# Lymphatus/caesium-clt

Measured on AMD Instinct MI355X. Metric: megapixels/sec JPEG q=80 1920x1080 batch, higher is better.
Workload: dtype int32

## Files before the change

### caesium-clt_amd/csrc/k_aclist.hip

```cpp
#include "kernels.h"
#include "wave.h"
#include "tok_bits.h"

namespace csh {

#define CSH_LP_WORDS 1024

__device__ __forceinline__ static uint32_t lbitlen(uint32_t v) { return 32u - uint32_t(__clz(v)); }
__device__ __forceinline__ static int lwave() { return int(threadIdx.x) / CSP_WAVE_THREADS; }

#define CSH_NZ_HALF 16
__device__ __forceinline__ static uint4 nz_load(const EncCtx &c, const NzSet &S, uint32_t u, int bx, int by, uint32_t oct) {
    uint4 q; q.x = q.y = q.z = q.w = 0u;
    if (u < S.nunits) {
        const int b = by * S.bw + bx;
        q = *reinterpret_cast<const uint4 *>(c.coef + (size_t(S.tile_base) + size_t(b >> 6)) * CSH_TILE_I16 + size_t((b & 63) * CSH_BLK_STRIDE) + size_t(oct) * CSH_OCT_STRIDE);
    }
    return q;
}
__device__ __forceinline__ static uint32_t nz_mask8(const uint4 &q, uint32_t oct) {
    uint32_t m = 0;
    m |= (q.x & 0xFFFFu) ? 1u : 0u;   m |= (q.x >> 16) ? 2u : 0u;
    m |= (q.y & 0xFFFFu) ? 4u : 0u;   m |= (q.y >> 16) ? 8u : 0u;
    m |= (q.z & 0xFFFFu) ? 16u : 0u;  m |= (q.z >> 16) ? 32u : 0u;
// ... 279 lines not shown
    const uint32_t idx = blockIdx.x * 4u + uint32_t(wv);
    if (idx >= c.nlist_runs) return;
    const uint32_t cs0 = c.list_runs[idx];
    const SlotRec r = c.slots[cs0];
    if (c.work_active && !c.work_active[r.work]) return;
    const uint32_t nrun = run_chunks(c, r);
    const uint64_t lbase = c.nzlists[r.nzlist].base;
    ListSlot nx = list_chunk(c, lbase, r.nzrec);
    uint32_t *hist = &s_hist[wv][0][0], *flag = s_flag[wv];
    LFOR(l) {
        uint4 zero; zero.x = zero.y = zero.z = zero.w = 0u;
        for (int i = 4 * l; i < 1024; i += 256) *reinterpret_cast<uint4 *>(hist + i) = zero;
        if (l < 16) flag[l] = 0u;
    }
    CSP_WAVE_SYNC();
    const uint32_t Ss = r.Ss, Se = r.Se;
    LV<uint32_t> freq[4];
    LFOR(l) { freq[0][l] = 0u; freq[1][l] = 0u; freq[2][l] = 0u; freq[3][l] = 0u; }
    LV<uint32_t> x0, x1, x2, x3;
    bool ahead = false;
    for (uint32_t ci = 0; ci < nrun; ci++) {
        const ListSlot ls = nx;
        const bool more = ci + 1u < nrun;
        if (more) nx = list_chunk(c, lbase, r.nzrec + ci + 1u);
        if (!ahead) LFOR(l) list_load4(ls, 4u * uint32_t(l), x0[l], x1[l], x2[l], x3[l]);
        ahead = false;
        uint32_t carry = CSH_NZ_END;
        LV<uint32_t> raw;
        LFOR(l) raw[l] = 0u;
        for (uint32_t g0 = 0; g0 < ls.n; g0 += 256) {
            const LV<uint32_t> e0 = x0, e1 = x1, e2 = x2, e3 = x3;
            if (g0 + 256u < ls.n) LFOR(l) list_load4(ls, g0 + 256u + 4u * uint32_t(l), x0[l], x1[l], x2[l], x3[l]);
            else if (more) { LFOR(l) list_load4(nx, 4u * uint32_t(l), x0[l], x1[l], x2[l], x3[l]); ahead = true; }
            const LV<uint32_t> p0 = lprev(e3, carry);
            carry = llast(e3);
            LFOR(l) {
                uint32_t *h = hist + 256 * (l & 3);
                const uint32_t e[4] = {e0[l], e1[l], e2[l], e3[l]}, p[4] = {p0[l], e0[l], e1[l], e2[l]};
                CSH_UNROLL
                for (int q = 0; q < 4; q++) {
                    const NzEvent v = nz_event(e[q], p[q], Ss, Se);
                    if (v.coded) {
                        atomicAdd(&h[((v.run & 15u) << 4) | v.size], 1u);
                        if (v.run >> 4) atomicAdd(&h[0xF0], v.run >> 4);
                        raw[l] += v.size;
                    } else if (v.term) {
                        if (v.has) atomicOr(&flag[v.blk >> 5], 1u << (v.blk & 31u));
                        if (v.eob) atomicOr(&flag[8u + (v.blk >> 5)], 1u << (v.blk & 31u));
                    }
                }
            }
        }
        CSP_WAVE_SYNC();
        const uint32_t rawbits = lsum32(raw);
        const uint32_t cs = cs0 + ci, j = r.j + ci, hist_row = r.hist_row + ci * uint32_t(r.ntables);
        hist_flush(hist, c.slot_hist + size_t(hist_row) * 256u, freq);
        LFOR(l) {
            if (l == 0) c.slot_raw[cs] = rawbits;
            if (l < 4 && j * 4u + uint32_t(l) < ((r.nunits_work + 63u) >> 6)) {
                c.sym_bits[r.word_base + j * 4u + uint32_t(l)] = uint64_t(flag[2 * l]) | (uint64_t(flag[2 * l + 1]) << 32);
                c.eob_bits[r.word_base + j * 4u + uint32_t(l)] = uint64_t(flag[8 + 2 * l]) | (uint64_t(flag[9 + 2 * l]) << 32);
            }
        }
        CSP_WAVE_SYNC();
        LFOR(l) if (l < 16) flag[l] = 0u;
        CSP_WAVE_SYNC();
    }
    freq_flush(c.tables[r.table_base].freq, freq);
}

__device__ __forceinline__ static void lor_bits(uint32_t *words, uint64_t pos, uint32_t v, uint32_t n) {
    v &= n >= 32 ? 0xFFFFFFFFu : ((1u << n) - 1u);
    const uint64_t t = uint64_t(v) << (64u - n - uint32_t(pos & 31u));
    const uint32_t hi = uint32_t(t >> 32), lo = uint32_t(t);
    if (hi) atomicOr(words + (pos >> 5), hi);
    if (lo) atomicOr(words + (pos >> 5) + 1, lo);
}
__global__ void __launch_bounds__(256) k_list_pack(EncCtx c) {
    CSH_SHARED alignas(16) uint32_t s_win[4][CSH_LP_WORDS];
    CSH_SHARED uint32_t s_lut[4][256];
    CSH_SHARED uint16_t s_eob[4][256];
    const int wv = int(uni(uint32_t(lwave())));
    const uint32_t idx = blockIdx.x * 4u + uint32_t(wv);
    if (idx >= c.nlist_runs) return;
    const uint32_t cs0 = c.list_runs[idx];
    const SlotRec r = c.slots[cs0];
    if (c.work_active && !c.work_active[r.work]) return;
    const ScanWork &w = c.work[r.work];
    if (w.no_room) { LFOR(l) if (l == 0) c.status[w.image] = 20200; return; }
    const uint32_t nrun = run_chunks(c, r);
    const uint64_t lbase = c.nzlists[r.nzlist].base;
    ListSlot nx = list_chunk(c, lbase, r.nzrec);
    const uint64_t scan0 = c.chunk_off[r.first_chunk];
    const uint64_t raw_bit0 = w.raw_off * 8 + (c.chunk_off[cs0] - scan0);
    uint32_t pad = 0;
    if (r.j + nrun == r.nch) { const uint64_t total = c.chunk_off[r.first_chunk + r.nch] - scan0; pad = uint32_t((8 - (total & 7)) & 7); }
    uint32_t *buf = s_win[wv], *lut = s_lut[wv];
    uint16_t *eobrun = s_eob[wv];
    LFOR(l) {
        for (int i = l; i < 256; i += 64) lut[i] = c.tables[r.table_base].lut[i];
        uint4 zero; zero.x = zero.y = zero.z = zero.w = 0u;
        for (int i = 4 * l; i < CSH_LP_WORDS; i += 256) *reinterpret_cast<uint4 *>(buf + i) = zero;
    }
    CSP_WAVE_SYNC();
    uint32_t *out = c.raw + (raw_bit0 >> 5);
    uint64_t pos = raw_bit0 & 31u;
    uint32_t ww = 0;
    bool first_flush = true;
    const uint32_t Ss = r.Ss, Se = r.Se;
    const uint32_t zrl = lut[0xF0], zc = zrl & 0xFFFFu, zl = zrl >> 16;
    LV<uint32_t> x0, x1, x2, x3;
    bool ahead = false;
    for (uint32_t ci = 0; ci < nrun; ci++) {
        const ListSlot ls = nx;
        const bool more = ci + 1u < nrun;
        if (more) nx = list_chunk(c, lbase, r.nzrec + ci + 1u);
#ifdef CSH_EMUL
        {
            const uint64_t want = (raw_bit0 & 31u) + (c.chunk_off[cs0 + ci] - c.chunk_off[cs0]);
            if (c.overflow[1] ? pos > want : pos != want) { fprintf(stderr, "k_list_pack: chunk %u of a run does not start where the one before it ended\n", ci); abort(); }
        }
#endif
        CSP_WAVE_SYNC();
        {
            const uint32_t u0 = r.unit0 + 256u * ci, left = r.nunits_work - 256u * (r.j + ci), nun = left < 256u ? left : 256u;
            LFOR(l) for (int i = l; i < 256; i += 64) eobrun[i] = uint32_t(i) < nun ? c.eobrun[u0 + uint32_t(i)] : uint16_t(0);
        }
        CSP_WAVE_SYNC();
        if (!ahead) LFOR(l) list_load4(ls, 4u * uint32_t(l), x0[l], x1[l], x2[l], x3[l]);
        ahead = false;
        uint32_t carry = CSH_NZ_END;
        const uint32_t cpad = more ? 0u : pad;
        const uint32_t n_ext = ls.n + (cpad ? 1u : 0u);
        for (uint32_t g0 = 0; g0 < n_ext; g0 += 256) {
            const LV<uint32_t> e0 = x0, e1 = x1, e2 = x2, e3 = x3;
            if (g0 + 256u < n_ext) LFOR(l) list_load4(ls, g0 + 256u + 4u * uint32_t(l), x0[l], x1[l], x2[l], x3[l]);
            else if (more) { LFOR(l) list_load4(nx, 4u * uint32_t(l), x0[l], x1[l], x2[l], x3[l]); ahead = true; }
            const LV<uint32_t> p0 = lprev(e3, carry);
            carry = llast(e3);
            LV<uint32_t> v0, v1, v2, v3, n0, n1, n2, n3, z, len;
            LFOR(l) {
                const uint32_t e[4] = {e0[l], e1[l], e2[l], e3[l]}, p[4] = {p0[l], e0[l], e1[l], e2[l]};
                uint32_t v[4], n[4], zz = 0, ln = 0;
                CSH_UNROLL
                for (int q = 0; q < 4; q++) {
                    v[q] = 0; n[q] = 0;
                    const uint32_t g = g0 + 4u * uint32_t(l) + uint32_t(q);
                    const NzEvent ev = nz_event(e[q], p[q], Ss, Se);
                    if (g >= ls.n) { if (cpad && g == ls.n) { v[q] = (1u << cpad) - 1u; n[q] = cpad; } }
                    else if (ev.coded) {
                        const uint32_t t = lut[((ev.run & 15u) << 4) | ev.size];
                        v[q] = ((t & 0xFFFFu) << ev.size) | ev.bits; n[q] = (t >> 16) + ev.size;
                        zz |= (ev.run >> 4) << (2 * q);
                        ln += (ev.run >> 4) * zl;
                    } else if (ev.term) {
                        const uint32_t run = eobrun[ev.blk];
                        if (run) {
                            const uint32_t nb = lbitlen(run) - 1u, t = lut[nb << 4];
                            v[q] = ((t & 0xFFFFu) << nb) | (run & ((1u << nb) - 1u)); n[q] = (t >> 16) + nb;
                        }
                    }
                    ln += n[q];
                }
                v0[l] = v[0]; v1[l] = v[1]; v2[l] = v[2]; v3[l] = v[3]; n0[l] = n[0]; n1[l] = n[1]; n2[l] = n[2]; n3[l] = n[3]; z[l] = zz; len[l] = ln;
            }
            uint32_t tot;
            const LV<uint32_t> ex = lscan(len, tot);
            LFOR(l) {
                uint64_t at = pos + ex[l] - uint64_t(ww) * 32u;
                const uint32_t v[4] = {v0[l], v1[l], v2[l], v3[l]}, n[4] = {n0[l], n1[l], n2[l], n3[l]};
                CSH_UNROLL
                for (int q = 0; q < 4; q++) {
                    for (uint32_t t = (z[l] >> (2 * q)) & 3u; t; t--) { lor_bits(buf, at, zc, zl); at += zl; }
                    if (n[q]) { lor_bits(buf, at, v[q], n[q]); at += n[q]; }
                }
            }
            pos += tot;
            const uint32_t done = uint32_t(pos >> 5) - ww;
            if (done > CSH_LP_WORDS - 640) {
                CSP_WAVE_SYNC();
                LFOR(l) for (uint32_t q = uint32_t(l); q < done; q += 64) {
                    const uint32_t v = buf[q];
                    if (first_flush && q == 0) { if (v) atomicOr(out + ww, v); } else out[ww + q] = v;
                }
                const uint32_t partial = buf[done];
                CSP_WAVE_SYNC();
                LFOR(l) for (int q = l; q < CSH_LP_WORDS; q += 64) buf[q] = (q == 0) ? partial : 0u;
                CSP_WAVE_SYNC();
                ww += done; first_flush = false;
            }
        }
    }
#ifdef CSH_EMUL
    {
        const uint64_t want = (raw_bit0 & 31u) + (c.chunk_off[cs0 + nrun] - c.chunk_off[cs0]) + pad;
        if (c.overflow[1] ? pos > want : pos != want) { fprintf(stderr, "k_list_pack: a run does not end where its sizes say\n"); abort(); }
    }
#endif
    CSP_WAVE_SYNC();
    const uint32_t last = uint32_t((pos + 31) >> 5) - ww;
    LFOR(l) for (uint32_t q = uint32_t(l); q < last; q += 64) {
        const uint32_t v = buf[q];
        if ((first_flush && q == 0) || q == last - 1) { if (v) atomicOr(out + ww + q, v); } else out[ww + q] = v;
    }
}

struct RefCarry { uint32_t runH, runN, base, prevN, prevNZ; };
__device__ __forceinline__ static uint32_t ref_isN(uint32_t e, uint32_t Ss, uint32_t Se) { const uint32_t k = e & 127u; return (k >= Ss && k <= Se && ((e >> 8) & 0x7FFFu) == 1u) ? 1u : 0u; }
__device__ __forceinline__ static uint32_t ref_isH(uint32_t e, uint32_t Ss, uint32_t Se) { const uint32_t k = e & 127u; return (k >= Ss && k <= Se && ((e >> 8) & 0x7FFFu) >= 2u) ? 1u : 0u; }
__device__ __forceinline__ static uint32_t ref_same(uint32_t key, uint32_t blk) { return (key >> 6) == blk + 1u ? (key & 63u) : 0u; }
template <bool WITH_ZQ>
__device__ __forceinline__ static void ref_step(const LV<uint32_t> (&e)[4], uint32_t Ss, uint32_t Se, RefCarry &C, LV<uint32_t> (&hex)[4], LV<uint32_t> (&z)[4], LV<uint32_t> (&zp)[4],
                                                LV<uint32_t> (&zq)[4]) {
    LV<uint32_t> cnt;
    LFOR(l) {
        uint32_t s = 0;
        CSH_UNROLL
        for (int q = 0; q < 4; q++) s += ref_isH(e[q][l], Ss, Se) | (ref_isN(e[q][l], Ss, Se) << 16);
        cnt[l] = s;
    }
    uint32_t tot;
    const LV<uint32_t> ex = lscan(cnt, tot);
    LV<uint32_t> kb[4];
    LFOR(l) {
        uint32_t ph = C.runH + (ex[l] & 0xFFFFu), pn = C.runN + (ex[l] >> 16);
        CSH_UNROLL
        for (int q = 0; q < 4; q++) {
            kb[q][l] = (e[q][l] & CSH_NZ_END) ? ((ph << 14) | pn) + 1u : 0u;
            hex[q][l] = ph; z[q][l] = pn;
            ph += ref_isH(e[q][l], Ss, Se); pn += ref_isN(e[q][l], Ss, Se);
        }
    }
    C.runH += tot & 0xFFFFu; C.runN += tot >> 16;
    lscan_last4(kb, C.base);
    LFOR(l) {
        CSH_UNROLL
        for (int q = 0; q < 4; q++) {
            const uint32_t b = kb[q][l] ? kb[q][l] - 1u : 0u, blk = (e[q][l] >> 23) & 255u, nz = ref_isH(e[q][l], Ss, Se) | ref_isN(e[q][l], Ss, Se);
            const uint32_t h = hex[q][l] - (b >> 14), n = z[q][l] - (b & 0x3FFFu);
            hex[q][l] = h;
            z[q][l] = nz ? (e[q][l] & 127u) - Ss - h - n : 0u;
            const uint32_t key = ((blk + 1u) << 6) | z[q][l];
            zp[q][l] = ref_isN(e[q][l], Ss, Se) ? key : 0u;
            if (WITH_ZQ) zq[q][l] = nz ? key : 0u;
        }
    }
    lscan_last4(zp, C.prevN);
    if (WITH_ZQ) lscan_last4(zq, C.prevNZ);
    LFOR(l) {
        CSH_UNROLL
        for (int q = 0; q < 4; q++) {
            const uint32_t blk = (e[q][l] >> 23) & 255u;
            zp[q][l] = ref_same(zp[q][l], blk);
            if (WITH_ZQ) zq[q][l] = ref_same(zq[q][l], blk);
        }
    }
}
template <class TL, class TN>
__device__ __forceinline__ static uint32_t ref_step_tokens(const LV<uint32_t> (&e)[4], const LV<uint32_t> (&hex)[4], const LV<uint32_t> (&z)[4], const LV<uint32_t> (&zp)[4], LV<uint32_t> (&zq)[4],
                                                           uint32_t Ss, uint32_t Se, const TL *lastn, const TN *nh, uint32_t &curc, uint32_t *tk, uint32_t at, uint32_t limit) {
    LV<uint32_t> cur[4], nt;
    LFOR(l) {
        uint32_t s = 0;
        CSH_UNROLL
        for (int q = 0; q < 4; q++) {
            const uint32_t v = e[q][l], blk = (v >> 23) & 255u, lastk = uint32_t(lastn[blk]) >> 6, isN = ref_isN(v, Ss, Se);
            uint32_t nz = 0, n = 0;
            if ((isN | ref_isH(v, Ss, Se)) && (v & 127u) <= lastk) { nz = ((z[q][l] - zp[q][l]) >> 4) - ((zq[q][l] - zp[q][l]) >> 4); n = nz + isN; }
            cur[q][l] = n ? ((blk + 1u) << 6) | hex[q][l] : 0u;
            if ((v & CSH_NZ_END) && lastk != Se) n = 1u;
            zq[q][l] = nz | (n << 8);
            s += n;
        }
        nt[l] = s;
    }
    lscan_last4(cur, curc);
    uint32_t tot;
    const LV<uint32_t> ex = lscan(nt, tot);
    LFOR(l) {
        uint32_t o = at + ex[l];
        CSH_UNROLL
        for (int q = 0; q < 4; q++) {
            const uint32_t v = e[q][l], blk = (v >> 23) & 255u, nz = zq[q][l] & 255u, n = zq[q][l] >> 8;
            if (!n) continue;
            const uint32_t cu = ref_same(cur[q][l], blk);
            if (v & CSH_NZ_END) {
                if (o < limit) tk[o] = TK_EOB | (blk << 3) | ((uint32_t(nh[blk]) - cu) << 16) | (cu << 22);
                o++;
                continue;
            }
            uint32_t cnt = hex[q][l] - cu, from = cu;
            for (uint32_t t = 0; t < nz; t++) {
                if (o < limit) tk[o] = TK_REF | (blk << 3) | (cnt << 16) | (from << 22) | (1u << 28);
                o++; cnt = 0u; from = hex[q][l];
            }
            if (n > nz) {
                if (o < limit) tk[o] = TK_REF | (blk << 3) | (((z[q][l] - zp[q][l]) & 15u) << 11) | ((v & 128u) ? 0u : (1u << 15)) | (cnt << 16) | (from << 22);
                o++;
            }
        }
    }
    return tot;
}
template <bool TOKENS>
__global__ void __launch_bounds__(256, 5) k_list_refine(EncCtx c) {
    CSH_SHARED alignas(16) uint32_t s_hist[4][4][256];
    CSH_SHARED uint32_t s_lastn[4][256];
    CSH_SHARED uint32_t s_nh[4][256];
    CSH_SHARED uint32_t s_corr[4][256][2];
    const int wv = int(uni(uint32_t(lwave())));
    const uint32_t idx = blockIdx.x * 4u + uint32_t(wv);
    if (idx >= c.nref_runs) return;
    const uint32_t cs0 = c.ref_runs[idx];
    const SlotRec r = c.slots[cs0];
    if (c.work_active && !c.work_active[r.work]) return;
    const uint32_t nrun = run_chunks(c, r);
    const uint64_t lbase = c.nzlists[r.nzlist].base;
    ListSlot nx = list_chunk(c, lbase, r.nzrec);
    TokRegion rg;
    rg.base = 0; rg.cap = 0; rg.pad = 0;
    if (TOKENS) rg = c.regions[r.region];
    uint32_t *hist = &s_hist[wv][0][0], *lastn = s_lastn[wv], *nh = s_nh[wv], *corr = &s_corr[wv][0][0];
    LFOR(l) {
        uint4 zero; zero.x = zero.y = zero.z = zero.w = 0u;
        for (int i = 4 * l; i < 1024; i += 256) *reinterpret_cast<uint4 *>(hist + i) = zero;
    }
    const uint32_t Ss = r.Ss, Se = r.Se;
    LV<uint32_t> freq[4];
    LFOR(l) { freq[0][l] = 0u; freq[1][l] = 0u; freq[2][l] = 0u; freq[3][l] = 0u; }
    for (uint32_t ci = 0; ci < nrun; ci++) {
        const ListSlot ls = nx;
        if (ci + 1u < nrun) nx = list_chunk(c, lbase, r.nzrec + ci + 1u);
        const uint32_t cs = cs0 + ci, j = r.j + ci, unit0 = r.unit0 + 256u * ci, corr0 = r.corr0 + 256u * ci, hist_row = r.hist_row + ci * uint32_t(r.ntables);
        const uint32_t left = r.nunits_work - 256u * j, nun = left < 256u ? left : 256u;
        CSP_WAVE_SYNC();
        LFOR(l) for (int i = l; i < 256; i += 64) { lastn[i] = 0u; nh[i] = 0u; corr[2 * i] = 0u; corr[2 * i + 1] = 0u; }
        CSP_WAVE_SYNC();
        RefCarry C;
        C.runH = C.runN = C.base = C.prevN = C.prevNZ = 0u;
        LV<uint32_t> ntok;
        LFOR(l) ntok[l] = 0u;
        {
        LV<uint32_t> x[4];
        LFOR(l) list_load4(ls, 4u * uint32_t(l), x[0][l], x[1][l], x[2][l], x[3][l]);
        for (uint32_t g0 = 0; g0 < ls.n; g0 += 256) {
            LV<uint32_t> e[4], hex[4], z[4], zp[4], zq[4];
            LFOR(l) { e[0][l] = x[0][l]; e[1][l] = x[1][l]; e[2][l] = x[2][l]; e[3][l] = x[3][l]; }
            if (g0 + 256u < ls.n) LFOR(l) list_load4(ls, g0 + 256u + 4u * uint32_t(l), x[0][l], x[1][l], x[2][l], x[3][l]);
            ref_step<false>(e, Ss, Se, C, hex, z, zp, zq);
            LFOR(l) {
                uint32_t *h = hist + 256 * (l & 3);
                CSH_UNROLL
                for (int q = 0; q < 4; q++) {
                    const uint32_t v = e[q][l], blk = (v >> 23) & 255u;
                    if (ref_isH(v, Ss, Se)) {
                        atomicMax(&nh[blk], hex[q][l] + 1u);
                        if (v & 0x100u) atomicOr(&corr[2u * blk + (hex[q][l] >> 5)], 0x80000000u >> (hex[q][l] & 31u));
                    } else if (ref_isN(v, Ss, Se)) {
                        const uint32_t zr = z[q][l] - zp[q][l];
                        atomicMax(&lastn[blk], ((v & 127u) << 6) | hex[q][l]);
                        atomicAdd(&h[((zr & 15u) << 4) | 1u], 1u);
                        if (zr >> 4) atomicAdd(&h[0xF0], zr >> 4);
                        ntok[l] += 1u + (zr >> 4);
                    }
                }
            }
        }
        }
        CSP_WAVE_SYNC();
        for (uint32_t w4 = 0; w4 < 4; w4++) {
            LFOR(l) {
                const uint32_t i = 64u * w4 + uint32_t(l);
                if (i < nun) {
                    const uint32_t ln = lastn[i];
                    if (ls.n && (ln >> 6) != Se) ntok[l] += 1u;
                    c.tail[unit0 + i] = uint8_t(nh[i] - (ln & 63u));
                    c.corr[corr0 + i] = (uint64_t(corr[2u * i]) << 32) | corr[2u * i + 1u];
                    if (!TOKENS) c.lastn[corr0 + i] = uint16_t(ln);
                }
            }
            const uint64_t ms = lballot([&](int b) { const uint32_t i = 64u * w4 + uint32_t(b); return i < nun && lastn[i] != 0u; });
            const uint64_t me = lballot([&](int b) { const uint32_t i = 64u * w4 + uint32_t(b); return i < nun && (lastn[i] >> 6) != Se; });
            LFOR(l) if (l == 0 && j * 4u + w4 < ((r.nunits_work + 63u) >> 6)) { c.sym_bits[r.word_base + j * 4u + w4] = ms; c.eob_bits[r.word_base + j * 4u + w4] = me; }
        }
        const uint32_t total = lsum32(ntok);
        hist_flush(hist, c.slot_hist + size_t(hist_row) * 256u, freq);
        LFOR(l) if (l == 0) c.slot_raw[cs] = C.runN + C.runH;
        if (c.stats_only || !TOKENS) continue;
        uint32_t rel = 0;
        LFOR(l) if (l == 0) rel = atomicAdd(&c.tok_cursor[r.region], total);
        rel = uni(rel);
        const bool ok = uint64_t(rel) + total <= rg.cap;
        LFOR(l) {
            if (l < 4) { c.tok_off[cs * 4u + uint32_t(l)] = rg.base + rel; c.chunk_ntok[cs * 4u + uint32_t(l)] = (ok && l == 0) ? total : 0u; }
            if (l == 0 && !ok) c.overflow[1] = 1;
        }
        if (!ok) continue;
        uint32_t *tk = c.tokens + rg.base + rel;
        C.runH = C.runN = C.base = C.prevN = C.prevNZ = 0u;
        uint32_t curc = 0, at = 0;
        for (uint32_t g0 = 0; g0 < ls.n; g0 += 256) {
            LV<uint32_t> e[4], hex[4], z[4], zp[4], zq[4];
            LFOR(l) list_load4(ls, g0 + 4u * uint32_t(l), e[0][l], e[1][l], e[2][l], e[3][l]);
            ref_step<true>(e, Ss, Se, C, hex, z, zp, zq);
            at += ref_step_tokens(e, hex, z, zp, zq, Ss, Se, lastn, nh, curc, tk, at, total);
        }
#ifdef CSH_EMUL
        if (at != total) { fprintf(stderr, "k_list_refine: pass 2 made %u tokens, pass 1 counted %u\n", at, total); abort(); }
#endif
    }
    freq_flush(c.tables[r.table_base].freq, freq);
}

#define CSH_RP_TOKENS 704
#define CSH_RP_SUB 64
#define CSH_RP_WORDS 256
#define CSH_RP_STEP 192
__global__ void __launch_bounds__(256, 5) k_list_refine_pack(EncCtx c) {
    CSH_SHARED alignas(16) uint32_t s_win[4][CSH_RP_WORDS];
    CSH_SHARED uint32_t s_lut[4][256];
    CSH_SHARED uint64_t s_corr[4][256];
    CSH_SHARED uint16_t s_eob[4][256];
    CSH_SHARED uint16_t s_lastn[4][256];
    CSH_SHARED uint8_t s_nh[4][256];
    CSH_SHARED uint32_t s_tok[4][CSH_RP_TOKENS];
    const int wv = int(uni(uint32_t(lwave())));
    const uint32_t idx = blockIdx.x * 4u + uint32_t(wv);
    if (idx >= c.nref_runs) return;
    const uint32_t cs0 = c.ref_runs[idx];
    const SlotRec r = c.slots[cs0];
    if (c.work_active && !c.work_active[r.work]) return;
    const ScanWork &w = c.work[r.work];
    if (w.no_room) { LFOR(l) if (l == 0) c.status[w.image] = 20200; return; }
    const uint32_t nrun = run_chunks(c, r);
    const uint64_t lbase = c.nzlists[r.nzlist].base;
    ListSlot nx = list_chunk(c, lbase, r.nzrec);
    const uint64_t scan0 = c.chunk_off[r.first_chunk];
    const uint64_t raw_bit0 = w.raw_off * 8 + (c.chunk_off[cs0] - scan0);
    uint32_t pad = 0;
    if (r.j + nrun == r.nch) { const uint64_t total = c.chunk_off[r.first_chunk + r.nch] - scan0; pad = uint32_t((8 - (total & 7)) & 7); }
    uint32_t *buf = s_win[wv], *lut = s_lut[wv];
    uint64_t *corr = s_corr[wv];
    uint16_t *eobrun = s_eob[wv], *lastn = s_lastn[wv];
    uint8_t *nh = s_nh[wv];
    uint32_t *tok = s_tok[wv];
    LFOR(l) {
        for (int i = l; i < 256; i += 64) lut[i] = c.tables[r.table_base].lut[i];
        uint4 zero; zero.x = zero.y = zero.z = zero.w = 0u;
        for (int i = 4 * l; i < CSH_RP_WORDS; i += 256) *reinterpret_cast<uint4 *>(buf + i) = zero;
    }
    CSP_WAVE_SYNC();
    TokenCtx x;
    x.lut = lut; x.lut_stride = 256; x.eobrun = eobrun; x.corr = corr;
    uint32_t *out = c.raw + (raw_bit0 >> 5);
    uint64_t pos = raw_bit0 & 31u;
    uint32_t ww = 0;
    bool first_flush = true;
    const uint32_t Ss = r.Ss, Se = r.Se;
    for (uint32_t ci = 0; ci < nrun; ci++) {
        const ListSlot ls = nx;
        const bool more = ci + 1u < nrun;
        if (more) nx = list_chunk(c, lbase, r.nzrec + ci + 1u);
#ifdef CSH_EMUL
        {
            const uint64_t want = (raw_bit0 & 31u) + (c.chunk_off[cs0 + ci] - c.chunk_off[cs0]);
            if (c.overflow[1] ? pos > want : pos != want) { fprintf(stderr, "k_list_refine_pack: chunk %u of a run does not start where the one before it ended\n", ci); abort(); }
        }
#endif
        CSP_WAVE_SYNC();
        {
            const uint32_t u0 = r.unit0 + 256u * ci, corr0 = r.corr0 + 256u * ci, left = r.nunits_work - 256u * (r.j + ci), nun = left < 256u ? left : 256u;
            LFOR(l) for (int i = l; i < 256; i += 64) {
                const bool in = uint32_t(i) < nun;
                const uint32_t ln = in ? uint32_t(c.lastn[corr0 + uint32_t(i)]) : 0u;
                eobrun[i] = in ? c.eobrun[u0 + uint32_t(i)] : uint16_t(0);
                corr[i] = in ? c.corr[corr0 + uint32_t(i)] : uint64_t(0);
                lastn[i] = uint16_t(ln);
                nh[i] = in ? uint8_t(uint32_t(c.tail[u0 + uint32_t(i)]) + (ln & 63u)) : uint8_t(0);
            }
        }
        CSP_WAVE_SYNC();
        LV<uint32_t> xn[4];
        LFOR(l) list_load4(ls, 4u * uint32_t(l), xn[0][l], xn[1][l], xn[2][l], xn[3][l]);
        RefCarry C;
        C.runH = C.runN = C.base = C.prevN = C.prevNZ = 0u;
        uint32_t curc = 0;
        for (uint32_t g0 = 0; g0 < ls.n; g0 += 256) {
            uint32_t ntok;
            {
                LV<uint32_t> e[4], hex[4], z[4], zp[4], zq[4];
                LFOR(l) { e[0][l] = xn[0][l]; e[1][l] = xn[1][l]; e[2][l] = xn[2][l]; e[3][l] = xn[3][l]; }
                if (g0 + 256u < ls.n) LFOR(l) list_load4(ls, g0 + 256u + 4u * uint32_t(l), xn[0][l], xn[1][l], xn[2][l], xn[3][l]);
                ref_step<true>(e, Ss, Se, C, hex, z, zp, zq);
                ntok = ref_step_tokens(e, hex, z, zp, zq, Ss, Se, lastn, nh, curc, tok, 0u, uint32_t(CSH_RP_TOKENS));
            }
#ifdef CSH_EMUL
            if (ntok > CSH_RP_TOKENS) { fprintf(stderr, "k_list_refine_pack: a step of %u tokens\n", ntok); abort(); }
#endif
            CSP_WAVE_SYNC();
            for (uint32_t s0 = 0; s0 < ntok; s0 += CSH_RP_SUB) {
                LV<uint32_t> t, pv[3], pn[3], slow, len;
                LFOR(l) {
                    const uint32_t i = s0 + uint32_t(l);
                    t[l] = i < ntok ? tok[i] : uint32_t(TK_RAW);
                    uint32_t v, n;
                    slow[l] = token_main<2>(t[l], x, v, n) ? 0u : 1u;
                    pv[0][l] = v; pn[0][l] = n; pv[1][l] = 0u; pn[1][l] = 0u; pv[2][l] = 0u; pn[2][l] = 0u;
                }
                if (lballot([&](int b) { return slow[b] != 0u; })) {
                    LFOR(l) {
                        const Pieces p = token_pieces<2>(t[l], x);
                        CSH_UNROLL
                        for (int k = 0; k < 3; k++) { pv[k][l] = p.v[k]; pn[k][l] = p.n[k]; }
                    }
                }
                LFOR(l) len[l] = pn[0][l] + pn[1][l] + pn[2][l];
                uint32_t tot;
                const LV<uint32_t> ex = lscan(len, tot);
                LFOR(l) {
                    uint64_t at = pos + ex[l] - uint64_t(ww) * 32u;
                    CSH_UNROLL
                    for (int k = 0; k < 3; k++) if (pn[k][l]) { lor_bits(buf, at, pv[k][l], pn[k][l]); at += pn[k][l]; }
                }
                pos += tot;
                const uint32_t done = uint32_t(pos >> 5) - ww;
                if (done > CSH_RP_WORDS - CSH_RP_STEP) {
                    CSP_WAVE_SYNC();
                    LFOR(l) for (uint32_t q = uint32_t(l); q < done; q += 64) {
                        const uint32_t v = buf[q];
                        if (first_flush && q == 0) { if (v) atomicOr(out + ww, v); } else out[ww + q] = v;
                    }
                    const uint32_t partial = buf[done];
                    CSP_WAVE_SYNC();
                    LFOR(l) for (int q = l; q < CSH_RP_WORDS; q += 64) buf[q] = (q == 0) ? partial : 0u;
                    CSP_WAVE_SYNC();
                    ww += done; first_flush = false;
                }
            }
            CSP_WAVE_SYNC();
        }
    }
    if (pad) { LFOR(l) if (l == 0) lor_bits(buf, pos - uint64_t(ww) * 32u, (1u << pad) - 1u, pad); pos += pad; }
#ifdef CSH_EMUL
    {
        const uint64_t want = (raw_bit0 & 31u) + (c.chunk_off[cs0 + nrun] - c.chunk_off[cs0]) + pad;
        if (c.overflow[1] ? pos > want : pos != want) { fprintf(stderr, "k_list_refine_pack: a run does not end where its sizes say\n"); abort(); }
    }
#endif
    CSP_WAVE_SYNC();
    const uint32_t last = uint32_t((pos + 31) >> 5) - ww;
    LFOR(l) for (uint32_t q = uint32_t(l); q < last; q += 64) {
        const uint32_t v = buf[q];
        if ((first_flush && q == 0) || q == last - 1) { if (v) atomicOr(out + ww + q, v); } else out[ww + q] = v;
    }
}

__global__ void k_reset_works(ScanWork *work, int nwork) {
    const int j = int(blockIdx.x * blockDim.x + threadIdx.x);
    if (j >= nwork) return;
    work[j].out_off = 0xFFFFFFFFu; work[j].raw_bytes = 0; work[j].hdr_bytes = 0; work[j].ff_bytes = 0; work[j].no_room = 0;
}

void launch_nzlist(hipStream_t st, const EncCtx &c) {
    if (!c.nnzchunks) return;
    if (c.nz_build) CSH_LAUNCH_PHASED(k_nzlist, 3, dim3(c.nnzchunks), dim3(2 * CSP_WAVE_THREADS), st, c);
    if (c.nz_filter) CSH_LAUNCH(k_nzfilter, dim3(c.nnzchunks), dim3(CSP_WAVE_THREADS), st, c);
}
void launch_list_stats(hipStream_t st, const EncCtx &c) { if (c.nlist_runs) CSH_LAUNCH(k_list_stats, dim3((c.nlist_runs + 3) / 4), dim3(4 * CSP_WAVE_THREADS), st, c); }
void launch_list_refine(hipStream_t st, const EncCtx &c) {
    if (!c.nref_runs) return;
    if (c.ref_pack) CSH_LAUNCH(k_list_refine<false>, dim3((c.nref_runs + 3) / 4), dim3(4 * CSP_WAVE_THREADS), st, c);
    else CSH_LAUNCH(k_list_refine<true>, dim3((c.nref_runs + 3) / 4), dim3(4 * CSP_WAVE_THREADS), st, c);
}
void launch_list_refine_pack(hipStream_t st, const EncCtx &c) { if (c.nref_runs && c.ref_pack) CSH_LAUNCH(k_list_refine_pack, dim3((c.nref_runs + 3) / 4), dim3(4 * CSP_WAVE_THREADS), st, c); }
void launch_list_pack(hipStream_t st, const EncCtx &c) { if (c.nlist_runs) CSH_LAUNCH(k_list_pack, dim3((c.nlist_runs + 3) / 4), dim3(4 * CSP_WAVE_THREADS), st, c); }
__global__ void __launch_bounds__(64) k_make_slots(const ScanWork *works, uint32_t nworks, const EncScan *script, const NzList *nzlists, SlotRec *slots, uint32_t *slot_work, uint32_t *list_slots,
                                                   uint32_t *tok_slots, uint32_t *ref_slots, uint32_t *list_runs, uint32_t *ref_runs, uint32_t list_run) {
    const uint32_t wi = blockIdx.x;
    if (wi >= nworks) return;
    const ScanWork &w = works[wi];
    const EncScan &e = script[w.scan];
    const uint32_t nch = (w.nunits + 255u) / 256u;
    const bool prog_ac = e.Ss > 0 && !e.sequential, has_list = w.list != 0xFFFFFFFFu;
    const bool ref_list = has_list && prog_ac && e.Ah;
    const bool listed = has_list && !ref_list;
    for (uint32_t j = threadIdx.x; j < nch; j += blockDim.x) {
        SlotRec r;
        r.work = wi; r.j = j; r.nch = nch; r.first_chunk = w.first_chunk; r.unit0 = w.unit_base + 256u * j;
        r.nun = w.nunits - 256u * j < 256u ? w.nunits - 256u * j : 256u; r.table_base = w.table_base; r.ntables = uint16_t(e.ntables);
        r.flags = uint16_t((prog_ac ? 1 : 0) | (prog_ac && e.Ah ? 2 : 0) | (listed ? 4 : 0) | (ref_list ? 8 : 0));
        r.hist_row = w.hist_row0 + j * uint32_t(e.ntables);
        r.word_base = w.word_base; r.unit_base = w.unit_base; r.nunits_work = w.nunits;
        r.Ss = uint8_t(e.Ss); r.Se = uint8_t(e.Se); r.Ah = uint8_t(e.Ah); r.Al = uint8_t(e.Al); r.corr0 = w.corr_base == 0xFFFFFFFFu ? 0u : w.corr_base + 256u * j;
        r.nzlist = has_list ? w.list : 0u; r.nzrec = has_list ? nzlists[w.list].chunk0 + j : 0u; r.region = ref_list ? w.region : 0u;
        slots[w.first_chunk + j] = r;
        slot_work[w.first_chunk + j] = wi;
        if (w.ls_base != 0xFFFFFFFFu) (listed ? list_slots : tok_slots)[w.ls_base + j] = w.first_chunk + j;
        if (ref_list) ref_slots[w.rs_base + j] = w.first_chunk + j;
        if (listed && j % list_run == 0u) list_runs[w.lr_base + j / list_run] = w.first_chunk + j;
        if (ref_list && j % list_run == 0u) ref_runs[w.rr_base + j / list_run] = w.first_chunk + j;
    }
}
__global__ void __launch_bounds__(64) k_rebind_slots(const ScanWork *works, uint32_t nworks, const NzList *nzlists, SlotRec *slots) {
    const uint32_t wi = blockIdx.x;
    if (wi >= nworks) return;
    const ScanWork &w = works[wi];
    if (w.list == 0xFFFFFFFFu) return;
    const uint32_t nch = (w.nunits + 255u) / 256u, chunk0 = nzlists[w.list].chunk0;
    for (uint32_t j = threadIdx.x; j < nch; j += blockDim.x) { slots[w.first_chunk + j].nzlist = w.list; slots[w.first_chunk + j].nzrec = chunk0 + j; }
}
void launch_rebind_slots(hipStream_t st, const ScanWork *works, uint32_t nworks, const NzList *nzlists, SlotRec *slots) {
    if (nworks) CSH_LAUNCH(k_rebind_slots, dim3(nworks), dim3(64), st, works, nworks, nzlists, slots);
}
void launch_make_slots(hipStream_t st, const ScanWork *works, uint32_t nworks, const EncScan *script, const NzList *nzlists, SlotRec *slots, uint32_t *slot_work, uint32_t *list_slots,
                       uint32_t *tok_slots, uint32_t *ref_slots, uint32_t *list_runs, uint32_t *ref_runs, uint32_t list_run) {
    if (!nworks) return;
    CSH_LAUNCH(k_make_slots, dim3(nworks), dim3(64), st, works, nworks, script, nzlists, slots, slot_work, list_slots, tok_slots, ref_slots, list_runs, ref_runs, list_run);
}

void launch_reset_works(hipStream_t st, ScanWork *work, int nwork) { if (nwork) CSH_LAUNCH(k_reset_works, dim3((nwork + 255) / 256), dim3(256), st, work, nwork); }

}
```

### caesium-clt_amd/csrc/tok_bits.h

```cpp
#pragma once
#include "kernels.h"

namespace csh {

struct Pieces { uint32_t v[3], n[3]; };
struct TokenCtx {
    const uint32_t *lut;
    uint32_t lut_stride;
    const uint16_t *eobrun;
    const uint64_t *corr;
};
#define CSH_LUT_STRIDE uint32_t(sizeof(DevEncTable) / 4)
__device__ __forceinline__ static void corr_pieces(Pieces &p, uint64_t corr, uint32_t t) {
    const uint32_t cnt = (t >> 16) & 63u, cur = (t >> 22) & 63u;
    if (!cnt) return;
    const uint64_t bits = (corr << cur) >> (64u - cnt);
    if (cnt > 32) { p.v[1] = uint32_t(bits >> 32); p.n[1] = cnt - 32; p.v[2] = uint32_t(bits); p.n[2] = 32; }
    else { p.v[2] = uint32_t(bits); p.n[2] = cnt; }
}
template <int MODE = 0>
__device__ __forceinline__ static Pieces token_pieces(uint32_t t, const TokenCtx &x) {
    Pieces p;
    p.v[0] = p.v[1] = p.v[2] = 0; p.n[0] = p.n[1] = p.n[2] = 0;
    uint32_t kind = t & 7u;
    if (MODE == 1) { if (kind == TK_RAW) return p; kind = kind == TK_ACF ? uint32_t(TK_ACF) : uint32_t(TK_EOB); }
    if (MODE == 2) { if (kind == TK_RAW) return p; kind = kind == TK_REF ? uint32_t(TK_REF) : uint32_t(TK_EOB); }
    if (MODE == 3) kind = kind == TK_SYM ? uint32_t(TK_SYM) : uint32_t(TK_RAW);
    if (kind == TK_SYM) {
        const uint32_t e = x.lut[((t >> 11) & 3u) * x.lut_stride + ((t >> 3) & 255u)], nr = (t >> 13) & 15u;
        p.v[0] = ((e & 0xFFFFu) << nr) | (t >> 17); p.n[0] = (e >> 16) + nr;
    } else if (kind == TK_RAW) { p.v[0] = t >> 17; p.n[0] = (t >> 13) & 15u; }
    else if (kind == TK_ACF) {
        const uint32_t r = (t >> 3) & 63u, nb = (t >> 9) & 15u, zr = r >> 4;
        if (zr) {
            const uint32_t z = x.lut[0xF0], zc = z & 0xFFFFu, zl = z >> 16;
            p.v[0] = zc; p.n[0] = zl;
            if (zr > 1) { p.v[0] = (zc << zl) | zc; p.n[0] = 2 * zl; }
            if (zr > 2) { p.v[1] = zc; p.n[1] = zl; }
        }
        const uint32_t e = x.lut[((r & 15u) << 4) | nb];
        p.v[2] = ((e & 0xFFFFu) << nb) | ((t >> 13) & 0xFFFFu); p.n[2] = (e >> 16) + nb;
    } else if (kind == TK_REF) {
        const uint32_t unit = (t >> 3) & 255u;
        if (t & (1u << 28)) { const uint32_t e = x.lut[0xF0]; p.v[0] = e & 0xFFFFu; p.n[0] = e >> 16; }
        else { const uint32_t e = x.lut[(((t >> 11) & 15u) << 4) | 1u]; p.v[0] = ((e & 0xFFFFu) << 1) | ((t >> 15) & 1u); p.n[0] = (e >> 16) + 1; }
        if ((t >> 16) & 63u) corr_pieces(p, x.corr[unit], t);
    } else {
        const uint32_t unit = (t >> 3) & 255u;
        const uint32_t run = x.eobrun[unit];
        if (run) {
            const uint32_t nb = 31u - uint32_t(__clz(run));
            const uint32_t e = x.lut[nb << 4];
            p.v[0] = ((e & 0xFFFFu) << nb) | (run & ((1u << nb) - 1u)); p.n[0] = (e >> 16) + nb;
        }
        if ((t >> 16) & 63u) corr_pieces(p, x.corr[unit], t);
    }
    return p;
}
template <int MODE>
__device__ __forceinline__ static bool token_main(uint32_t t, const TokenCtx &x, uint32_t &v, uint32_t &n) {
    v = 0; n = 0;
    const uint32_t kind = t & 7u;
    if (kind == TK_RAW) { v = t >> 17; n = (t >> 13) & 15u; return true; }
    if (MODE == 3) {
        const uint32_t e = x.lut[((t >> 11) & 3u) * x.lut_stride + ((t >> 3) & 255u)], nr = (t >> 13) & 15u;
        v = ((e & 0xFFFFu) << nr) | (t >> 17); n = (e >> 16) + nr;
        return true;
    }
    if (MODE == 1 && kind == TK_ACF) {
        const uint32_t r = (t >> 3) & 63u, nb = (t >> 9) & 15u;
        if (r >> 4) return false;
        const uint32_t e = x.lut[(r << 4) | nb];
        v = ((e & 0xFFFFu) << nb) | ((t >> 13) & 0xFFFFu); n = (e >> 16) + nb;
        return true;
    }
    const uint32_t unit = (t >> 3) & 255u, cnt = (t >> 16) & 63u, cur = (t >> 22) & 63u;
    if (MODE == 2 && kind == TK_REF) {
        if (t & (1u << 28)) { const uint32_t e = x.lut[0xF0]; v = e & 0xFFFFu; n = e >> 16; }
        else { const uint32_t e = x.lut[(((t >> 11) & 15u) << 4) | 1u]; v = ((e & 0xFFFFu) << 1) | ((t >> 15) & 1u); n = (e >> 16) + 1; }
    } else {
        const uint32_t run = x.eobrun[unit];
        if (run) {
            const uint32_t nb = 31u - uint32_t(__clz(run));
            const uint32_t e = x.lut[nb << 4];
            v = ((e & 0xFFFFu) << nb) | (run & ((1u << nb) - 1u)); n = (e >> 16) + nb;
        }
    }
    if (MODE == 2 && cnt) {
        if (n + cnt > 32) return false;
        const uint32_t bits = uint32_t((x.corr[unit] << cur) >> (64u - cnt));
        v = (n ? (v << cnt) : 0u) | bits; n += cnt;
    }
    return true;
}

}
```

Measured before the change: 49230.

## Shrink refinement-scan LDS histograms and LUT, chunk token staging for occupancy

In k_list_refine, each wave's refinement histogram shrinks from four 256-word copies to four 32-word copies, because a refinement scan only uses the EOBRUN/ZRL and (run,1) symbols. A new flush packs those counts back into the 256-entry row layout. In k_list_refine_pack, the LUT is compacted to a 32-entry refinement-code table and the per-wave token staging buffer shrinks from 704 to 256 tokens. A step producing more tokens is now handled by replaying ref_step over the same 256 coefficients in several rounds. Together these cut LDS use per block so launch bounds can rise to 6 and 7 blocks per CU, at the cost of recomputing steps that overflow the smaller buffer.

```diff
diff --git a/caesium-clt_amd/csrc/k_aclist.hip b/caesium-clt_amd/csrc/k_aclist.hip
--- a/caesium-clt_amd/csrc/k_aclist.hip
+++ b/caesium-clt_amd/csrc/k_aclist.hip
@@ -605,9 +605,24 @@
     }
     return tot;
 }
+#define CSH_RH_WORDS 32
+__device__ __forceinline__ static void ref_hist_flush(uint32_t *hist, uint16_t *row, LV<uint32_t> (&freq)[4]) {
+    LFOR(l) {
+        uint32_t zrl = 0, run = 0;
+        CSH_UNROLL
+        for (int cpy = 0; cpy < 4; cpy++) {
+            uint32_t *h = hist + CSH_RH_WORDS * cpy;
+            if ((l & 3) == 0) { run += h[l >> 2]; h[l >> 2] = 0u; }
+            if (l == 60) { zrl += h[16]; h[16] = 0u; }
+        }
+        uint2 o; o.x = (zrl & 0xFFFFu) | (run << 16); o.y = 0u;
+        *reinterpret_cast<uint2 *>(row + 4 * l) = o;
+        freq[0][l] += zrl; freq[1][l] += run;
+    }
+}
 template <bool TOKENS>
-__global__ void __launch_bounds__(256, 5) k_list_refine(EncCtx c) {
-    CSH_SHARED alignas(16) uint32_t s_hist[4][4][256];
+__global__ void __launch_bounds__(256, 6) k_list_refine(EncCtx c) {
+    CSH_SHARED uint32_t s_hist[4][4][CSH_RH_WORDS];
     CSH_SHARED uint32_t s_lastn[4][256];
     CSH_SHARED uint32_t s_nh[4][256];
     CSH_SHARED uint32_t s_corr[4][256][2];
@@ -624,10 +639,7 @@
     rg.base = 0; rg.cap = 0; rg.pad = 0;
     if (TOKENS) rg = c.regions[r.region];
     uint32_t *hist = &s_hist[wv][0][0], *lastn = s_lastn[wv], *nh = s_nh[wv], *corr = &s_corr[wv][0][0];
-    LFOR(l) {
-        uint4 zero; zero.x = zero.y = zero.z = zero.w = 0u;
-        for (int i = 4 * l; i < 1024; i += 256) *reinterpret_cast<uint4 *>(hist + i) = zero;
-    }
+    LFOR(l) for (int i = l; i < 4 * CSH_RH_WORDS; i += 64) hist[i] = 0u;
     const uint32_t Ss = r.Ss, Se = r.Se;
     LV<uint32_t> freq[4];
     LFOR(l) { freq[0][l] = 0u; freq[1][l] = 0u; freq[2][l] = 0u; freq[3][l] = 0u; }
@@ -652,7 +664,7 @@
             if (g0 + 256u < ls.n) LFOR(l) list_load4(ls, g0 + 256u + 4u * uint32_t(l), x[0][l], x[1][l], x[2][l], x[3][l]);
             ref_step<false>(e, Ss, Se, C, hex, z, zp, zq);
             LFOR(l) {
-                uint32_t *h = hist + 256 * (l & 3);
+                uint32_t *h = hist + CSH_RH_WORDS * (l & 3);
                 CSH_UNROLL
                 for (int q = 0; q < 4; q++) {
                     const uint32_t v = e[q][l], blk = (v >> 23) & 255u;
@@ -662,8 +674,8 @@
                     } else if (ref_isN(v, Ss, Se)) {
                         const uint32_t zr = z[q][l] - zp[q][l];
                         atomicMax(&lastn[blk], ((v & 127u) << 6) | hex[q][l]);
-                        atomicAdd(&h[((zr & 15u) << 4) | 1u], 1u);
-                        if (zr >> 4) atomicAdd(&h[0xF0], zr >> 4);
+                        atomicAdd(&h[zr & 15u], 1u);
+                        if (zr >> 4) atomicAdd(&h[16], zr >> 4);
                         ntok[l] += 1u + (zr >> 4);
                     }
                 }
@@ -687,7 +699,7 @@
             LFOR(l) if (l == 0 && j * 4u + w4 < ((r.nunits_work + 63u) >> 6)) { c.sym_bits[r.word_base + j * 4u + w4] = ms; c.eob_bits[r.word_base + j * 4u + w4] = me; }
         }
         const uint32_t total = lsum32(ntok);
-        hist_flush(hist, c.slot_hist + size_t(hist_row) * 256u, freq);
+        ref_hist_flush(hist, c.slot_hist + size_t(hist_row) * 256u, freq);
         LFOR(l) if (l == 0) c.slot_raw[cs] = C.runN + C.runH;
         if (c.stats_only || !TOKENS) continue;
         uint32_t rel = 0;
@@ -715,13 +727,14 @@
     freq_flush(c.tables[r.table_base].freq, freq);
 }
 
-#define CSH_RP_TOKENS 704
+#define CSH_RP_STEP_TOKENS 648
+#define CSH_RP_TOKENS 256
 #define CSH_RP_SUB 64
 #define CSH_RP_WORDS 256
 #define CSH_RP_STEP 192
-__global__ void __launch_bounds__(256, 5) k_list_refine_pack(EncCtx c) {
+__global__ void __launch_bounds__(256, 7) k_list_refine_pack(EncCtx c) {
     CSH_SHARED alignas(16) uint32_t s_win[4][CSH_RP_WORDS];
-    CSH_SHARED uint32_t s_lut[4][256];
+    CSH_SHARED uint32_t s_lut[4][CSH_REF_CODES];
     CSH_SHARED uint64_t s_corr[4][256];
     CSH_SHARED uint16_t s_eob[4][256];
     CSH_SHARED uint16_t s_lastn[4][256];
@@ -748,13 +761,13 @@
     uint8_t *nh = s_nh[wv];
     uint32_t *tok = s_tok[wv];
     LFOR(l) {
-        for (int i = l; i < 256; i += 64) lut[i] = c.tables[r.table_base].lut[i];
+        if (l < CSH_REF_CODES) lut[l] = c.tables[r.table_base].lut[((uint32_t(l) & 15u) << 4) | (uint32_t(l) >> 4)];
         uint4 zero; zero.x = zero.y = zero.z = zero.w = 0u;
         for (int i = 4 * l; i < CSH_RP_WORDS; i += 256) *reinterpret_cast<uint4 *>(buf + i) = zero;
     }
     CSP_WAVE_SYNC();
     TokenCtx x;
-    x.lut = lut; x.lut_stride = 256; x.eobrun = eobrun; x.corr = corr;
+    x.lut = lut; x.lut_stride = CSH_REF_CODES; x.eobrun = eobrun; x.corr = corr;
     uint32_t *out = c.raw + (raw_bit0 >> 5);
     uint64_t pos = raw_bit0 & 31u;
     uint32_t ww = 0;
@@ -789,30 +802,39 @@
         C.runH = C.runN = C.base = C.prevN = C.prevNZ = 0u;
         uint32_t curc = 0;
         for (uint32_t g0 = 0; g0 < ls.n; g0 += 256) {
+            const RefCarry C0 = C;
+            const uint32_t curc0 = curc;
+            for (uint32_t t0 = 0;; t0 += CSH_RP_TOKENS) {
             uint32_t ntok;
             {
                 LV<uint32_t> e[4], hex[4], z[4], zp[4], zq[4];
-                LFOR(l) { e[0][l] = xn[0][l]; e[1][l] = xn[1][l]; e[2][l] = xn[2][l]; e[3][l] = xn[3][l]; }
-                if (g0 + 256u < ls.n) LFOR(l) list_load4(ls, g0 + 256u + 4u * uint32_t(l), xn[0][l], xn[1][l], xn[2][l], xn[3][l]);
+                if (t0 == 0u) {
+                    LFOR(l) { e[0][l] = xn[0][l]; e[1][l] = xn[1][l]; e[2][l] = xn[2][l]; e[3][l] = xn[3][l]; }
+                    if (g0 + 256u < ls.n) LFOR(l) list_load4(ls, g0 + 256u + 4u * uint32_t(l), xn[0][l], xn[1][l], xn[2][l], xn[3][l]);
+                } else {
+                    C = C0; curc = curc0;
+                    LFOR(l) list_load4(ls, g0 + 4u * uint32_t(l), e[0][l], e[1][l], e[2][l], e[3][l]);
+                }
                 ref_step<true>(e, Ss, Se, C, hex, z, zp, zq);
-                ntok = ref_step_tokens(e, hex, z, zp, zq, Ss, Se, lastn, nh, curc, tok, 0u, uint32_t(CSH_RP_TOKENS));
+                ntok = ref_step_tokens(e, hex, z, zp, zq, Ss, Se, lastn, nh, curc, tok, 0u - t0, uint32_t(CSH_RP_TOKENS));
             }
 #ifdef CSH_EMUL
-            if (ntok > CSH_RP_TOKENS) { fprintf(stderr, "k_list_refine_pack: a step of %u tokens\n", ntok); abort(); }
+            if (ntok > CSH_RP_STEP_TOKENS) { fprintf(stderr, "k_list_refine_pack: a step of %u tokens\n", ntok); abort(); }
 #endif
             CSP_WAVE_SYNC();
-            for (uint32_t s0 = 0; s0 < ntok; s0 += CSH_RP_SUB) {
+            const uint32_t nround = ntok - t0 < uint32_t(CSH_RP_TOKENS) ? ntok - t0 : uint32_t(CSH_RP_TOKENS);
+            for (uint32_t s0 = 0; s0 < nround; s0 += CSH_RP_SUB) {
                 LV<uint32_t> t, pv[3], pn[3], slow, len;
                 LFOR(l) {
                     const uint32_t i = s0 + uint32_t(l);
-                    t[l] = i < ntok ? tok[i] : uint32_t(TK_RAW);
+                    t[l] = i < nround ? tok[i] : uint32_t(TK_RAW);
                     uint32_t v, n;
-                    slow[l] = token_main<2>(t[l], x, v, n) ? 0u : 1u;
+                    slow[l] = token_main<2, true>(t[l], x, v, n) ? 0u : 1u;
                     pv[0][l] = v; pn[0][l] = n; pv[1][l] = 0u; pn[1][l] = 0u; pv[2][l] = 0u; pn[2][l] = 0u;
                 }
                 if (lballot([&](int b) { return slow[b] != 0u; })) {
                     LFOR(l) {
-                        const Pieces p = token_pieces<2>(t[l], x);
+                        const Pieces p = token_pieces<2, true>(t[l], x);
                         CSH_UNROLL
                         for (int k = 0; k < 3; k++) { pv[k][l] = p.v[k]; pn[k][l] = p.n[k]; }
                     }
@@ -841,6 +863,8 @@
                 }
             }
             CSP_WAVE_SYNC();
+            if (t0 + uint32_t(CSH_RP_TOKENS) >= ntok) break;
+            }
         }
     }
     if (pad) { LFOR(l) if (l == 0) lor_bits(buf, pos - uint64_t(ww) * 32u, (1u << pad) - 1u, pad); pos += pad; }
diff --git a/caesium-clt_amd/csrc/tok_bits.h b/caesium-clt_amd/csrc/tok_bits.h
--- a/caesium-clt_amd/csrc/tok_bits.h
+++ b/caesium-clt_amd/csrc/tok_bits.h
@@ -18,8 +18,13 @@
     if (cnt > 32) { p.v[1] = uint32_t(bits >> 32); p.n[1] = cnt - 32; p.v[2] = uint32_t(bits); p.n[2] = 32; }
     else { p.v[2] = uint32_t(bits); p.n[2] = cnt; }
 }
-template <int MODE = 0>
+#define CSH_REF_CODES 32
+__device__ __forceinline__ static uint32_t ref_code_index(uint32_t s) { return (s >> 4) | ((s & 1u) << 4); }
+template <bool REF32>
+__device__ __forceinline__ static uint32_t ref_code(const TokenCtx &x, uint32_t s) { return x.lut[REF32 ? ref_code_index(s) : s]; }
+template <int MODE = 0, bool REF32 = false>
 __device__ __forceinline__ static Pieces token_pieces(uint32_t t, const TokenCtx &x) {
+    static_assert(!REF32 || MODE == 2, "the 32-entry table holds a refinement scan's codes only");
     Pieces p;
     p.v[0] = p.v[1] = p.v[2] = 0; p.n[0] = p.n[1] = p.n[2] = 0;
     uint32_t kind = t & 7u;
@@ -42,23 +47,24 @@
         p.v[2] = ((e & 0xFFFFu) << nb) | ((t >> 13) & 0xFFFFu); p.n[2] = (e >> 16) + nb;
     } else if (kind == TK_REF) {
         const uint32_t unit = (t >> 3) & 255u;
-        if (t & (1u << 28)) { const uint32_t e = x.lut[0xF0]; p.v[0] = e & 0xFFFFu; p.n[0] = e >> 16; }
-        else { const uint32_t e = x.lut[(((t >> 11) & 15u) << 4) | 1u]; p.v[0] = ((e & 0xFFFFu) << 1) | ((t >> 15) & 1u); p.n[0] = (e >> 16) + 1; }
+        if (t & (1u << 28)) { const uint32_t e = ref_code<REF32>(x, 0xF0u); p.v[0] = e & 0xFFFFu; p.n[0] = e >> 16; }
+        else { const uint32_t e = ref_code<REF32>(x, (((t >> 11) & 15u) << 4) | 1u); p.v[0] = ((e & 0xFFFFu) << 1) | ((t >> 15) & 1u); p.n[0] = (e >> 16) + 1; }
         if ((t >> 16) & 63u) corr_pieces(p, x.corr[unit], t);
     } else {
         const uint32_t unit = (t >> 3) & 255u;
         const uint32_t run = x.eobrun[unit];
         if (run) {
             const uint32_t nb = 31u - uint32_t(__clz(run));
-            const uint32_t e = x.lut[nb << 4];
+            const uint32_t e = ref_code<REF32>(x, nb << 4);
             p.v[0] = ((e & 0xFFFFu) << nb) | (run & ((1u << nb) - 1u)); p.n[0] = (e >> 16) + nb;
         }
         if ((t >> 16) & 63u) corr_pieces(p, x.corr[unit], t);
     }
     return p;
 }
-template <int MODE>
+template <int MODE, bool REF32 = false>
 __device__ __forceinline__ static bool token_main(uint32_t t, const TokenCtx &x, uint32_t &v, uint32_t &n) {
+    static_assert(!REF32 || MODE == 2, "the 32-entry table holds a refinement scan's codes only");
     v = 0; n = 0;
     const uint32_t kind = t & 7u;
     if (kind == TK_RAW) { v = t >> 17; n = (t >> 13) & 15u; return true; }
@@ -76,13 +82,13 @@
     }
     const uint32_t unit = (t >> 3) & 255u, cnt = (t >> 16) & 63u, cur = (t >> 22) & 63u;
     if (MODE == 2 && kind == TK_REF) {
-        if (t & (1u << 28)) { const uint32_t e = x.lut[0xF0]; v = e & 0xFFFFu; n = e >> 16; }
-        else { const uint32_t e = x.lut[(((t >> 11) & 15u) << 4) | 1u]; v = ((e & 0xFFFFu) << 1) | ((t >> 15) & 1u); n = (e >> 16) + 1; }
+        if (t & (1u << 28)) { const uint32_t e = ref_code<REF32>(x, 0xF0u); v = e & 0xFFFFu; n = e >> 16; }
+        else { const uint32_t e = ref_code<REF32>(x, (((t >> 11) & 15u) << 4) | 1u); v = ((e & 0xFFFFu) << 1) | ((t >> 15) & 1u); n = (e >> 16) + 1; }
     } else {
         const uint32_t run = x.eobrun[unit];
         if (run) {
             const uint32_t nb = 31u - uint32_t(__clz(run));
-            const uint32_t e = x.lut[nb << 4];
+            const uint32_t e = ref_code<REF32>(x, nb << 4);
             v = ((e & 0xFFFFu) << nb) | (run & ((1u << nb) - 1u)); n = (e >> 16) + nb;
         }
     }
```

New measurement: 50000 (median of 6 runs). 1.02x the previous value.
